# Kitware/SMQTK-Indexing

Measured on AMD Instinct MI355X. Metric: queries/sec, exact brute-force l2 kNN k=100 over 10000000x128 float32 (recall@100 = 1.0 by construction); scan HBM GB/s vs 8 TB/s peak, higher is better.
Workload: dtype f32 results (distances bit-identical to numpy float32); filter arithmetic int8 MFMA (i32 accumulation, measured per-row error bound), exact re-rank f32

## Files before the change

### smqtk_indexing_amd/csrc/sq_dense_exact.hpp

```cpp
#pragma once
#include "sq_pairwise.hpp"
#include "sq_select.hpp"

namespace sq {

typedef float f32x4 __attribute__((ext_vector_type(4)));
typedef float f32x16 __attribute__((ext_vector_type(16)));

__device__ __forceinline__ float np_sqdist_f32(const float* __restrict__ x, const float* __restrict__ q, int d, int j8) {
    auto term = [x, q](int i) {
        const float t = __fsub_rn(x[i], q[i]);
        return __fmul_rn(t, t);
    };
    return np_pairwise_sum<float>(term, d, j8);
}

__device__ __forceinline__ float sqrt_rn_f32(float v) {
    return (float)sqrt((double)v);
}

__device__ __forceinline__ double cosine_dist_f64(double dot, double nx2, double nq2) {
    double c = __ddiv_rn(dot, __dmul_rn(sqrt(nq2), sqrt(nx2)));
    if (fabs(c) > 1.0) c = copysign(1.0, c);
    double dm = 1.0 - c;
// ... 747 lines not shown
        __syncthreads();
        if (threadIdx.x == 0) {
            double tot = 0.0;
            for (int w = 0; w < (T >> 6); ++w) tot += red[w];
            qn2_out[q] = tot;
            cnt[q] = 0u;
            if (q == 0) *oflag = 0u;
            for (int p = nq + q; p < nq_pad; p += gridDim.x) {
                qn2_out[p] = 0.0;
                thr_out[p] = -__builtin_inff();
                cnt[p] = 0u;
            }
        }
        __syncthreads();
    }
    __device__ __forceinline__ float operator()(int q, float t) const {
        if (traw_out) traw_out[q] = t;
        if (!(t < __builtin_inff())) return t;
        double slack;
        if (cosine) {
            slack = 2.0 * fb.eps_cos + 1e-8;
        } else {
            const double Q = qn2[q];
            const double gamma = 1.0 - 2.0 * fb.alpha - fb.eps_b;
            const double c = fb.beta * Q + (double)t;
            const double disc = Q + gamma * c;
            double rho = (sqrt(Q) + sqrt(disc > 0.0 ? disc : 0.0)) / gamma;
            double rho2 = rho * rho * (1.0 + 1e-9);
            if (rho2 > fb.xn2_max) rho2 = fb.xn2_max;
            slack = (2.0 * fb.alpha + fb.eps_b) * rho2 + 2.0 * fb.beta * Q + 4e-6 * fabs((double)t + Q);
        }
        float r = (float)((double)t + slack);
        if ((double)r < (double)t + slack) r = __uint_as_float(__float_as_uint(r) + (r >= 0.f ? 1 : -1));
        return r;
    }
};

struct DenseCallPtrs {
    const float* q;
    void* out_dist;
    long long* out_idx;
};

struct DenseFinalizeL2 {
    const u32* cnt;
    u32 cap;
    int kk;
    long long id_base;
    const float* thr;
    const double* qn2;
    double beta;
    int certify;
    float* out_dist;
    long long* out_idx;
    u32* status;
    u32* cnt_out;
    const u32* overflow;
    int q0;
    ExactGroup sel = ExactGroup{{0, 0, 0, 0, 0, 0, 0, 0}, 0};
    const int* qmap = nullptr;
    const float2* lin = nullptr;
    const u32* thr2k = nullptr;
    int cnt_shift = 0;
    const DenseCallPtrs* ind = nullptr;
    __device__ __forceinline__ void operator()(int ql, const u64* sorted, int k) const {
        const int q = qmap ? qmap[ql] : (sel.count ? sel.idx[ql] : q0 + ql);
        const int qa = qmap ? ql : q;
        float* out_dist = ind ? static_cast<float*>(ind->out_dist) : this->out_dist;
        long long* out_idx = ind ? ind->out_idx : this->out_idx;
        for (int j = threadIdx.x; j < k; j += blockDim.x) {
            const u64 key = sorted[j];
            const bool pad = key == ~0ull;
            out_dist[(long long)q * k + j] = pad ? __builtin_inff() : unordered_f32((u32)(key >> 32));
            out_idx[(long long)q * k + j] = pad ? -1ll : id_base + (long long)(key & 0xffffffffull);
        }
        if (threadIdx.x == 0) {
            u32 st = 0;
            const u32 c = cnt[(long long)((sel.count || qmap) ? ql : q) << cnt_shift];
            if (certify) {
                if (c > cap || (overflow && *overflow)) st |= 1u;
                if (c < (u32)kk) st |= 4u;
                if (st == 0 && certify == 1) {
                    const double dk = (double)unordered_f32((u32)(sorted[kk - 1] >> 32));
                    const u32 t2k = thr2k ? thr2k[(long long)qa << cnt_shift] : 0u;
                    const double t = t2k ? (double)unordered_f32(t2k) : (double)thr[qa];
                    const double lo2 = t + qn2[qa] * (1.0 - beta) - (lin ? (double)lin[qa].y : 0.0);
                    const double bound = lo2 > 0.0 ? sqrt(lo2) * (1.0 - 1e-6) : 0.0;
                    if (!(t == (double)__builtin_inff()) && !(dk < bound)) st |= 2u;
                }
            }
            status[q] = st;
            if (cnt_out) cnt_out[q] = c;
        }
    }
};

struct DenseFinalizeCos {
    const u32* cnt;
    u32 cap;
    int kk;
    long long id_base;
    const float* thr;
    double eps;
    int certify;
    double* out_dist;
    long long* out_idx;
    u32* status;
    u32* cnt_out;
    const u32* overflow;
    int q0;
    ExactGroup sel = ExactGroup{{0, 0, 0, 0, 0, 0, 0, 0}, 0};
    const float2* lin = nullptr;
    const u32* thr2k = nullptr;
    int cnt_shift = 0;
    const DenseCallPtrs* ind = nullptr;
    const int* qmap = nullptr;
    __device__ __forceinline__ void operator()(int ql, const K128* sorted, int k) const {
        const int q = qmap ? qmap[ql] : (sel.count ? sel.idx[ql] : q0 + ql);
        const int qa = qmap ? ql : q;
        double* out_dist = ind ? static_cast<double*>(ind->out_dist) : this->out_dist;
        long long* out_idx = ind ? ind->out_idx : this->out_idx;
        for (int j = threadIdx.x; j < k; j += blockDim.x) {
            const K128 key = sorted[j];
            const bool pad = key.hi == ~0ull && key.lo == ~0ull;
            out_dist[(long long)q * k + j] = pad ? (double)__builtin_inff() : unordered_f64(key.hi);
            out_idx[(long long)q * k + j] = pad ? -1ll : id_base + (long long)(key.lo & 0xffffffffull);
        }
        if (threadIdx.x == 0) {
            u32 st = 0;
            const u32 c = cnt[(long long)((sel.count || qmap) ? ql : q) << cnt_shift];
            if (certify) {
                if (c > cap || (overflow && *overflow)) st |= 1u;
                if (c < (u32)kk) st |= 4u;
                if (st == 0 && certify == 1) {
                    const double dk = unordered_f64(sorted[kk - 1].hi);
                    const u32 t2k = thr2k ? thr2k[(long long)qa << cnt_shift] : 0u;
                    const double t = t2k ? (double)unordered_f32(t2k) : (double)thr[qa];
                    double smax = -t + (lin ? (double)lin[qa].y : eps);
                    smax = smax > 1.0 ? 1.0 : (smax < -1.0 ? -1.0 : smax);
                    const double bound = 2.0 * acos(smax) / 3.141592653589793 - 1e-9;
                    if (!(t == (double)__builtin_inff()) && !(dk < bound)) st |= 2u;
                }
            }
            status[q] = st;
            if (cnt_out) cnt_out[q] = c;
        }
    }
};

}
```

### smqtk_indexing_amd/csrc/sq_dense_i8.hpp

```cpp
#pragma once
#include "sq_dense_scan.hpp"

namespace sq {

typedef int i32x4 __attribute__((ext_vector_type(4)));
typedef int i32x16 __attribute__((ext_vector_type(16)));

template <int KS>
struct I8Geom {
    static constexpr int ROW_BYTES = KS * 32;
    static constexpr int UNIT_ROWS = KS == 4 ? 64 : 32;
    static constexpr int TILES = UNIT_ROWS / 32;
    static constexpr int UNIT_BYTES = UNIT_ROWS * ROW_BYTES;
    static constexpr int SLOT_BYTES = UNIT_BYTES + 256;
    static constexpr int WAVES = KS <= 8 ? 8 : 4;
    static constexpr int NSTAGE = 2;
    static constexpr int PIECES = UNIT_BYTES / 1024;
    static constexpr int SAMPLES_PER_UNIT = 2 * TILES;
};
static constexpr int I8_MAX_ROW_BYTES = 512;
__host__ __device__ constexpr int i8_row_bytes(int d) { return d <= 128 ? 128 : (d <= 256 ? 256 : 512); }
__host__ __device__ constexpr int i8_unit_rows(int row_bytes) { return row_bytes == 128 ? 64 : 32; }

__device__ __forceinline__ float i8_element(float v, const float* __restrict__ center, int k, bool cosine, double inv_norm) {
// ... 288 lines not shown
    par_out = make_float2((float)unit, real ? ef : 0.f);
    qn2_out = real ? Q : 0.0;
}

template <int EPL>
static __global__ __launch_bounds__(64) void dense8_prep_queries_kernel(const float* __restrict__ q, int nq, int d,
                                                                         const float* __restrict__ center, double dx, double r_max,
                                                                         double x_max, signed char* __restrict__ qs8,
                                                                         float2* __restrict__ par, double* __restrict__ qn2,
                                                                         float* __restrict__ thr, u32* __restrict__ cnt,
                                                                         u32* __restrict__ oflag, float* __restrict__ q_al, int ldq,
                                                                         const DenseCallPtrs* __restrict__ ind, int cosine, int plane_rows) {
    constexpr int row_bytes = EPL * 64;
    if (ind) q = ind->q;
    const int qi = blockIdx.x * 4 + (threadIdx.x >> 4), t = threadIdx.x & 15;
    if (t == 0) {
        thr[qi] = qi < nq ? -__builtin_inff() : __builtin_nanf("");
        cnt[qi] = 0u;
        if (qi == 0) *oflag = 0u;
    }
    if (qi < nq)
        for (int i = t; i < ldq; i += 16) q_al[(long long)qi * ldq + i] = i < d ? q[(long long)qi * d + i] : 0.f;
    float2 pr;
    double Q;
    dense8_prep_query_row<EPL>(q + (long long)qi * d, qi < nq, d, center, dx, r_max, x_max, cosine,
                               qs8 + (long long)qi * row_bytes, qs8 + (long long)(plane_rows + qi) * row_bytes, pr, Q);
    if (t == 0) {
        par[qi] = pr;
        qn2[qi] = Q;
    }
}

struct Dense8ThrPost {
    const float2* par;
    const double* qn2;
    __device__ __forceinline__ void prologue(int, double*) const {}
    __device__ __forceinline__ float operator()(int q, float t) const {
        if (!(t < __builtin_inff())) return t;
        if (!(par[q].y < __builtin_inff())) return __builtin_nanf("");
        const double tt = (double)t + 2.0 * (double)par[q].y + 4e-6 * fabs((double)t + qn2[q]);
        float r = (float)tt;
        if ((double)r < tt) r = __uint_as_float(__float_as_uint(r) + (r >= 0.f ? 1 : -1));
        return r;
    }
};

struct Dense8ScanArgs {
    const signed char* scan8;
    const float* nrow;
    long long n;
    long long n_units;
    const signed char* qs8;
    const float2* par;
    const float* thr;
    uint2* wave_out;
    u32* wave_cnt;
    u32 wave_cap;
    float* sample_out;
    long long ns;
    long long unit_step;
    long long n_sel;
    int nrb;
    int nt;
    long long nt_from_row;
    int nqt;
    int plane_rows;
    int debug;
    float* wave_score;
    u32* hist;
};

template <int KS>
__device__ __forceinline__ int i8_swz(int c, int r) {
    if constexpr (KS == 4) return c ^ ((r >> 1) & 7);
    return (c & ~15) | ((c & 15) ^ (r & 15));
}

enum { I8_EMIT = 0, I8_SAMPLE = 1, I8_LANEMIN = 2, I8_EMIT_H = 3 };

static constexpr int I8_HIST_BINS = 64;
static constexpr int I8_CNT_SHIFT = 5;
static constexpr int I8_HIST_WORDS = TILE_ROWS * I8_HIST_BINS + (TILE_ROWS << I8_CNT_SHIFT);

template <int WAVES>
__device__ __forceinline__ void dense8_hist_flush(u32* lds_hist, u32* __restrict__ ghist) {
    constexpr int PER = TILE_ROWS * I8_HIST_BINS / WAVES;
    const int lane = threadIdx.x & 63;
    const int wave = __builtin_amdgcn_readfirstlane(threadIdx.x >> 6);
#pragma unroll
    for (int i = 0; i < PER / 64; ++i) {
        const int b = wave * PER + i * 64 + lane;
        const u32 v = __hip_atomic_exchange(lds_hist + b, 0u, __ATOMIC_RELAXED, __HIP_MEMORY_SCOPE_WORKGROUP);
        if (v) __hip_atomic_fetch_add(ghist + b, v, __ATOMIC_RELAXED, __HIP_MEMORY_SCOPE_AGENT);
    }
}

template <int KS, int MODE>
__device__ __forceinline__ void dense8_stream(const Dense8ScanArgs& a, unsigned char* smem, const i32x4 (&bq)[KS], const i32x4 (&bl)[KS],
                                              float unit_lo, float thr_l, u32& wcount, float& smin, u32* lds_ticket,
                                              float inv_w_l = 0.f, u32* lds_hist = nullptr) {
    using G = I8Geom<KS>;
    constexpr bool SAMPLE = MODE == I8_SAMPLE || MODE == I8_LANEMIN;
    const int lane = threadIdx.x & 63;
    const int wave = __builtin_amdgcn_readfirstlane(threadIdx.x >> 6);
    const int r31 = lane & 31, h = lane >> 5;
    const u32 lds_base = (u32)(uintptr_t)smem;
    const u32 ring_base = lds_base + (u32)wave * (G::NSTAGE * G::SLOT_BYTES);
    const unsigned char* ring_ptr = smem + wave * (G::NSTAGE * G::SLOT_BYTES);
    const long long wave_id = (long long)blockIdx.x * G::WAVES + wave;
    const long long nwaves = (long long)a.nrb * G::WAVES;
    uint2* wout = a.wave_out + wave_id * a.wave_cap;
    float* wsc = MODE == I8_EMIT_H ? a.wave_score + wave_id * a.wave_cap : nullptr;
    u32* hist_l = MODE == I8_EMIT_H ? lds_hist + r31 * I8_HIST_BINS : nullptr;

    const long long wg_first = (long long)blockIdx.x * G::WAVES;
    auto take_unit = [&]() __attribute__((always_inline)) -> long long {
        u32 t = 0;
        if (lane == 0) t = __hip_atomic_fetch_add(lds_ticket, 1u, __ATOMIC_RELAXED, __HIP_MEMORY_SCOPE_WORKGROUP);
        t = (u32)__builtin_amdgcn_readfirstlane((int)t);
        const long long u = wg_first + (long long)(t % G::WAVES) + (long long)(t / G::WAVES) * nwaves;
        return u < a.n_sel ? u : -1ll;
    };
    const long long my_units = wave_id < a.n_sel ? (a.n_sel - wave_id + nwaves - 1) / nwaves : 0;
    u32 voff[G::PIECES];
#pragma unroll
    for (int j = 0; j < G::PIECES; ++j) {
        const int lin = j * 1024 + lane * 16;
        const int r = lin / G::ROW_BYTES, cpos = (lin % G::ROW_BYTES) >> 4;
        voff[j] = (u32)(r * G::ROW_BYTES + i8_swz<KS>(cpos, r) * 16);
    }
    const u32 voff_n = (u32)lane * 4u;
    static_assert(G::NSTAGE == 2, "two ring slots: the units in flight are sel_even / sel_odd");
    long long issued = 0, sel_even = -1, sel_odd = -1;
    bool more = true;
    auto issue_next = [&]() __attribute__((always_inline)) {
        if (!more) return;
        const long long sel = take_unit();
        if (sel < 0) {
            more = false;
            return;
        }
        if (issued & 1) sel_odd = sel; else sel_even = sel;
        const long long unit_idx = sel * a.unit_step;
        const long long row0 = unit_idx * G::UNIT_ROWS;
        const u32 dst = ring_base + (u32)(issued % G::NSTAGE) * G::SLOT_BYTES;
        const unsigned char* base = reinterpret_cast<const unsigned char*>(a.scan8) + row0 * G::ROW_BYTES;
#pragma unroll
        for (int j = 0; j < G::PIECES; ++j) {
            if (a.nt && row0 >= a.nt_from_row)
                glds16<true>(base, voff[j], dst + (u32)j * 1024);
            else
                glds16<false>(base, voff[j], dst + (u32)j * 1024);
        }
        glds4(a.nrow + row0, voff_n, dst + G::UNIT_BYTES);
        ++issued;
    };
    for (int p = 0; p < G::NSTAGE; ++p) issue_next();
    const int flush_every = (int)(my_units >> 3) > 0 ? (int)(my_units >> 3) : 1;
    int to_flush = flush_every;

    for (long long it = 0; it < issued; ++it) {
        const long long sel = (it & 1) ? sel_odd : sel_even;
        const long long unit_idx = sel * a.unit_step;
        const long long row0 = unit_idx * G::UNIT_ROWS;
        wait_units_in_flight<G::NSTAGE, G::PIECES + 1>((int)(issued - it - 1));
        const unsigned char* sl = ring_ptr + (it % G::NSTAGE) * G::SLOT_BYTES;
        constexpr int KH = KS == 16 ? 8 : KS;
        i32x4 av[G::TILES][KH];
        f32x4 nr[G::TILES][4];
#pragma unroll
        for (int t = 0; t < G::TILES; ++t) {
            const int r = 32 * t + r31;
#pragma unroll
            for (int s = 0; s < KH; ++s)
                av[t][s] = *reinterpret_cast<const i32x4*>(sl + r * G::ROW_BYTES + i8_swz<KS>(2 * s + h, r) * 16);
#pragma unroll
            for (int c = 0; c < 4; ++c) nr[t][c] = *reinterpret_cast<const f32x4*>(sl + G::UNIT_BYTES + (32 * t + 8 * c + 4 * h) * 4);
        }
        asm volatile("s_waitcnt lgkmcnt(0)" ::: "memory");
        if constexpr (KS != 16) issue_next();
#pragma unroll
        for (int t = 0; t < G::TILES; ++t) {
            i32x16 acc, acl;
#pragma unroll
            for (int i = 0; i < 16; ++i) acc[i] = acl[i] = 0;
#pragma unroll
            for (int s = 0; s < KH; ++s) {
                acc = __builtin_amdgcn_mfma_i32_32x32x32_i8(av[t][s], bq[s], acc, 0, 0, 0);
                acl = __builtin_amdgcn_mfma_i32_32x32x32_i8(av[t][s], bl[s], acl, 0, 0, 0);
            }
            if constexpr (KS == 16) {
#pragma unroll
                for (int s = 0; s < KH; ++s)
                    av[t][s] = *reinterpret_cast<const i32x4*>(sl + r31 * G::ROW_BYTES + i8_swz<KS>(2 * (KH + s) + h, r31) * 16);
                asm volatile("s_waitcnt lgkmcnt(0)" ::: "memory");
                issue_next();
#pragma unroll
                for (int s = 0; s < KH; ++s) {
                    acc = __builtin_amdgcn_mfma_i32_32x32x32_i8(av[t][s], bq[KH + s], acc, 0, 0, 0);
                    acl = __builtin_amdgcn_mfma_i32_32x32x32_i8(av[t][s], bl[KH + s], acl, 0, 0, 0);
                }
            }
            if (a.debug & 1024) {
                if (acc[0] == 0x7fffffff && acl[5] == 0x7ffffffe) wcount += 1;
                continue;
            }
            float sc[16];
#pragma unroll
            for (int i = 0; i < 16; ++i) {
                float nv = nr[t][i >> 2][i & 3];
                if constexpr (SAMPLE) nv = nv == -__builtin_inff() ? __builtin_inff() : nv;
                sc[i] = __fmaf_rn((float)((acc[i] << 8) + acl[i]), unit_lo, nv);
            }
            float m = sc[0];
#pragma unroll
            for (int i = 1; i < 16; ++i) m = fminf(m, sc[i]);
            if constexpr (MODE == I8_LANEMIN) {
                smin = fminf(smin, m);
            } else if constexpr (MODE == I8_SAMPLE) {
                a.sample_out[(long long)r31 * a.ns + sel * G::SAMPLES_PER_UNIT + t * 2 + h] = m;
            } else {
                const u64 hit = __ballot(m <= thr_l);
                if (hit != 0) {
                    u32 mask = 0;
#pragma unroll
                    for (int i = 0; i < 16; ++i) mask |= (sc[i] <= thr_l ? 1u : 0u) << i;
                    const u64 bal = __ballot(mask != 0);
                    if (mask) {
                        const u32 pos = wcount + __builtin_amdgcn_mbcnt_hi((u32)(bal >> 32), __builtin_amdgcn_mbcnt_lo((u32)bal, 0u));
                        if (pos < a.wave_cap) {
                            wout[pos] = make_uint2((u32)(row0 + 32 * t + 4 * h), (mask << 16) | (u32)r31);
                            if constexpr (MODE == I8_EMIT_H) wsc[pos] = m;
                        }
                        if constexpr (MODE == I8_EMIT_H) {
                            if (m > -__builtin_inff()) {
                                const int bin = min((int)((thr_l - m) * inv_w_l), I8_HIST_BINS - 1);
                                __hip_atomic_fetch_add(hist_l + bin, 1u, __ATOMIC_RELAXED, __HIP_MEMORY_SCOPE_WORKGROUP);
                            }
                        }
                    }
                    wcount += (u32)__popcll(bal);
                }
            }
        }
        if constexpr (MODE == I8_EMIT_H) {
            if (--to_flush == 0) {
                to_flush = flush_every;
                dense8_hist_flush<G::WAVES>(lds_hist, a.hist);
            }
        }
    }
}

template <int KS>
__device__ __forceinline__ void dense8_load_planes(const signed char* planes, i32x4 (&bq)[KS], i32x4 (&bl)[KS]) {
    using G = I8Geom<KS>;
    const int lane = threadIdx.x & 63, r31 = lane & 31, h = lane >> 5;
#pragma unroll
    for (int s = 0; s < KS; ++s) {
        bq[s] = *reinterpret_cast<const i32x4*>(planes + r31 * G::ROW_BYTES + (2 * s + h) * 16);
        bl[s] = *reinterpret_cast<const i32x4*>(planes + (TILE_ROWS + r31) * G::ROW_BYTES + (2 * s + h) * 16);
    }
#pragma unroll
    for (int s = 0; s < KS; ++s) asm volatile("" : "+v"(bq[s]), "+v"(bl[s]));
}

template <int KS, bool SAMPLE>
__global__ __launch_bounds__(I8Geom<KS>::WAVES * 64, KS == 16 ? 1 : 2) void dense8_scan_kernel(Dense8ScanArgs a) {
    using G = I8Geom<KS>;
    extern __shared__ __attribute__((aligned(16))) unsigned char smem[];
    const int lane = threadIdx.x & 63;
    const int wave = __builtin_amdgcn_readfirstlane(threadIdx.x >> 6);
    const int r31 = lane & 31;
    i32x4 bq[KS], bl[KS];
    dense8_load_planes<KS>(a.qs8, bq, bl);
    float unit_lo = a.par[r31].x * 0.00390625f;
    float thr_l = SAMPLE ? 0.f : a.thr[r31];
    asm volatile("" : "+v"(unit_lo), "+v"(thr_l));
    u32 wcount = 0;
    float smin = 0.f;
    __shared__ u32 s_unit_ticket;
    if (threadIdx.x == 0) s_unit_ticket = 0u;
    __syncthreads();
    dense8_stream<KS, SAMPLE ? I8_SAMPLE : I8_EMIT>(a, smem, bq, bl, unit_lo, thr_l, wcount, smin, &s_unit_ticket);
    if constexpr (!SAMPLE) {
        if (lane == 0) {
            const long long wave_id = (long long)blockIdx.x * G::WAVES + wave;
            a.wave_cnt[2 * wave_id] = wcount;
            a.wave_cnt[2 * wave_id + 1] = 0u;
        }
    }
}


struct Dense8HeadArgs {
    Dense8ScanArgs s;
    const float* q;
    int nq, d;
    const float* center;
    double dx, r_max, x_max;
    int cosine;
    double* qn2;
    u32* cnt;
    u32* oflag;
    float* q_al;
    int ldq;
    const DenseCallPtrs* ind;
    float* lane_min;
    int keep;
    int kk;
};

template <int VM, int NQ>
__device__ __forceinline__ void wave_kth_smallest(const float* __restrict__ vals, long long stride, int M, int k, float (&out)[NQ]) {
    const int lane = threadIdx.x & 63;
    constexpr u32 KINF = 0xff800000u;
    u32 key[NQ][VM];
    u32 prefix[NQ];
    u32 xall = 0u;
#pragma unroll
    for (int n = 0; n < NQ; ++n) {
        u32 kmin = KINF, kmax = 0u;
#pragma unroll
        for (int j = 0; j < VM; ++j) {
            const int i = j * 64 + lane;
            u32 kv = ordered_f32(vals[n * stride + (i < M ? i : 0)]);
            kv = (i < M && kv < KINF) ? kv : KINF;
            key[n][j] = kv;
            kmin = kv < kmin ? kv : kmin;
            kmax = kv > kmax ? kv : kmax;
        }
        for (int o = 32; o > 0; o >>= 1) {
            const u32 a = (u32)__shfl_xor((int)kmin, o), b = (u32)__shfl_xor((int)kmax, o);
            kmin = a < kmin ? a : kmin;
            kmax = b > kmax ? b : kmax;
        }
        prefix[n] = __builtin_amdgcn_readfirstlane(kmin);
        xall |= __builtin_amdgcn_readfirstlane(kmin ^ kmax);
    }
    if (xall != 0u) {
        const int top = 31 - __clz((int)xall);
#pragma unroll
        for (int n = 0; n < NQ; ++n) prefix[n] &= ~((2u << top) - 1u);
        for (int b = top; b >= 0; --b) {
#pragma unroll
            for (int n = 0; n < NQ; ++n) {
                const u32 cand = prefix[n] | ((1u << b) - 1u);
                u32 c = 0;
#pragma unroll
                for (int j = 0; j < VM; ++j) c += (u32)__popcll(__ballot(key[n][j] <= cand));
                if (c < (u32)k) prefix[n] |= 1u << b;
            }
        }
    }
#pragma unroll
    for (int n = 0; n < NQ; ++n) {
        float r = unordered_f32(prefix[n]);
        if (prefix[n] >= KINF) {
            u32 c = 0;
#pragma unroll
            for (int j = 0; j < VM; ++j) c += (u32)__popcll(__ballot(key[n][j] < KINF));
            if (c < (u32)k) r = __builtin_inff();
        }
        out[n] = r;
    }
}

template <int KS>
__global__ __launch_bounds__(I8Geom<KS>::WAVES * 64, KS == 16 ? 1 : 2) void dense8_head_kernel(Dense8HeadArgs ha) {
    using G = I8Geom<KS>;
    constexpr int VB = G::WAVES * 2;
    extern __shared__ __attribute__((aligned(16))) unsigned char smem[];
    __shared__ float2 s_par[TILE_ROWS];
    __shared__ double s_qn2[TILE_ROWS];
    __shared__ float s_lm[TILE_ROWS][16];
    __shared__ u32 s_ticket, s_unit_ticket;
    if (threadIdx.x == 0) s_unit_ticket = 0u;
    const Dense8ScanArgs& a = ha.s;
    const int lane = threadIdx.x & 63;
    const int wave = __builtin_amdgcn_readfirstlane(threadIdx.x >> 6);
    const int r31 = lane & 31, h = lane >> 5;
    const float* q = ha.ind ? ha.ind->q : ha.q;
    const bool first = blockIdx.x == 0;
    signed char* planes = reinterpret_cast<signed char*>(smem);
#pragma unroll
    for (int rnd = 0; rnd < TILE_ROWS / (4 * G::WAVES); ++rnd) {
        const int qi = rnd * 4 * G::WAVES + wave * 4 + (lane >> 4);
        float2 pr;
        double Q;
        dense8_prep_query_row<KS / 2>(q + (long long)qi * ha.d, qi < ha.nq, ha.d, ha.center, ha.dx, ha.r_max, ha.x_max, ha.cosine,
                                      planes + qi * G::ROW_BYTES, planes + (TILE_ROWS + qi) * G::ROW_BYTES, pr, Q);
        if ((lane & 15) == 0) {
            s_par[qi] = pr;
            s_qn2[qi] = Q;
        }
        if (first) {
            if ((lane & 15) == 0) {
                const_cast<float2*>(a.par)[qi] = pr;
                ha.qn2[qi] = Q;
                ha.cnt[qi << I8_CNT_SHIFT] = 0u;
                if (qi == 0) ha.oflag[0] = 0u;
            }
            if (qi < ha.nq)
                for (int i = lane & 15; i < ha.ldq; i += 16) ha.q_al[(long long)qi * ha.ldq + i] = i < ha.d ? q[(long long)qi * ha.d + i] : 0.f;
        }
    }
    __syncthreads();
    i32x4 bq[KS], bl[KS];
    dense8_load_planes<KS>(planes, bq, bl);
    float unit_lo = s_par[r31].x * 0.00390625f;
    asm volatile("" : "+v"(unit_lo));
    if (first) {
        signed char* gp = const_cast<signed char*>(a.qs8);
        for (int i = threadIdx.x; i < 2 * TILE_ROWS * G::ROW_BYTES / 16; i += G::WAVES * 64)
            reinterpret_cast<uint4*>(gp)[i] = reinterpret_cast<const uint4*>(planes)[i];
        for (int i = threadIdx.x; i < I8_HIST_WORDS; i += G::WAVES * 64) a.hist[i] = 0u;
    }
    asm volatile("s_waitcnt vmcnt(0) lgkmcnt(0)" ::: "memory");
    __syncthreads();
    u32 wcount = 0;
    float smin = __builtin_inff();
    if (!(a.debug & 4096)) dense8_stream<KS, I8_LANEMIN>(a, smem, bq, bl, unit_lo, 0.f, wcount, smin, &s_unit_ticket);
    s_lm[r31][(wave * 2 + h) & 15] = smin;
    if (VB < 16 && wave == 0 && h == 0)
        for (int i = VB; i < 16; ++i) s_lm[r31][i] = __builtin_inff();
    __syncthreads();
    const int nb = (int)gridDim.x, keep = ha.keep, M = nb * keep;
#pragma unroll
    for (int rnd = 0; rnd < TILE_ROWS / (4 * G::WAVES); ++rnd) {
        const int qi = rnd * 4 * G::WAVES + wave * 4 + (lane >> 4), l16 = lane & 15;
        float v = s_lm[qi][l16];
#pragma unroll
        for (int kk2 = 2; kk2 <= 16; kk2 <<= 1)
#pragma unroll
            for (int j = kk2 >> 1; j > 0; j >>= 1) {
                const float o = __shfl_xor(v, j);
                const bool up = (l16 & kk2) == 0, lower = (l16 & j) == 0;
                v = (lower == up) ? fminf(v, o) : fmaxf(v, o);
            }
        if (l16 < keep) ha.lane_min[(long long)qi * M + (long long)blockIdx.x * keep + l16] = v;
    }
    asm volatile("s_waitcnt vmcnt(0)" ::: "memory");
    __syncthreads();
    if (threadIdx.x == 0) {
        __threadfence();
        const u32 t = atomicAdd(&ha.oflag[1], 1u);
        if (t == gridDim.x - 1) {
            __threadfence();
            ha.oflag[1] = 0u;
        }
        s_ticket = t;
    }
    __syncthreads();
    if (s_ticket != gridDim.x - 1) return;
    float* thr = const_cast<float*>(a.thr);
    const Dense8ThrPost post{s_par, s_qn2};
#pragma unroll
    for (int rnd = 0; rnd < TILE_ROWS / (4 * G::WAVES); ++rnd) {
        const int q0 = rnd * 4 * G::WAVES + wave * 4;
        float ts[4] = {-__builtin_inff(), -__builtin_inff(), -__builtin_inff(), -__builtin_inff()};
        if (q0 < ha.nq && !(a.debug & 2048)) {
            const float* v = ha.lane_min + (long long)q0 * M;
            if (M <= 256)
                wave_kth_smallest<4, 4>(v, M, M, ha.kk, ts);
            else if (M <= 512)
                wave_kth_smallest<8, 4>(v, M, M, ha.kk, ts);
            else if (M <= 1024)
                wave_kth_smallest<16, 4>(v, M, M, ha.kk, ts);
            else {
#pragma unroll
                for (int j = 0; j < 4; ++j) {
                    float one[1];
                    wave_kth_smallest<32, 1>(v + (long long)j * M, M, M, ha.kk, one);
                    ts[j] = one[0];
                }
            }
        }
#pragma unroll
        for (int j = 0; j < 4; ++j) {
            const float t = q0 + j < ha.nq ? post(q0 + j, ts[j]) : __builtin_nanf("");
            if (lane == 0) thr[q0 + j] = t;
        }
    }
}

struct Dense8TailArgs {
    const float* db;
    long long ld;
    int d;
    const float* q_al;
    int ldq, nq;
    void* keys;
    u32* cnt;
    u32 cap;
    u32* overflow;
    const double* nx64;
    const double* nq64;
    int debug;
    const double* qn2;
    int kk;
    int tighten;
    long long* clk;
};
static constexpr int I8_TAIL_QROWS_BYTES = 32 * (156 + 4) * 4;
static constexpr int I8_TAIL_LIST = 2048;
static constexpr int I8_TAIL_RERANK_BYTES = I8_TAIL_QROWS_BYTES + 3 * RERANK_MAX_GROUP * 4 + 8 * 32 * RERANK_STAGE_STRIDE * 4;
static constexpr int I8_TAIL_LDS_BYTES = I8_TAIL_RERANK_BYTES + I8_TAIL_LIST * 8 + TILE_ROWS * 4 + 16;

template <int KS, bool COSINE>
__global__ __launch_bounds__(I8Geom<KS>::WAVES * 64, KS == 16 ? 1 : 2) void dense8_body_kernel(Dense8ScanArgs a, Dense8TailArgs ta) {
    using G = I8Geom<KS>;
    static_assert(I8_TAIL_LDS_BYTES <= G::WAVES * G::NSTAGE * G::SLOT_BYTES, "the re-rank works in the ring's LDS");
    extern __shared__ __attribute__((aligned(16))) unsigned char smem[];
    __shared__ u32 s_hist8[TILE_ROWS * I8_HIST_BINS];
    __shared__ u32 s_wcnt[G::WAVES];
    __shared__ u32 s_unit_ticket;
    __shared__ float s_thr1[TILE_ROWS], s_eq[TILE_ROWS];
    __shared__ double s_qn2b[TILE_ROWS];
    __shared__ float2 s_parb[TILE_ROWS];
    if (threadIdx.x == 0) s_unit_ticket = 0u;
    if (threadIdx.x < TILE_ROWS) {
        s_thr1[threadIdx.x] = a.thr[threadIdx.x];
        s_parb[threadIdx.x] = a.par[threadIdx.x];
        s_eq[threadIdx.x] = a.par[threadIdx.x].y;
        s_qn2b[threadIdx.x] = ta.qn2[threadIdx.x];
    }
    const int lane = threadIdx.x & 63;
    const int wave = __builtin_amdgcn_readfirstlane(threadIdx.x >> 6);
    const int r31 = lane & 31;
    for (int i = threadIdx.x; i < TILE_ROWS * I8_HIST_BINS; i += G::WAVES * 64) s_hist8[i] = 0u;
    long long* clk = ta.clk ? ta.clk + (long long)blockIdx.x * 8 : nullptr;
    if (clk && threadIdx.x == 0) {
        clk[0] = (long long)wall_clock64();
        clk[1] = 0x7fffffffffffffffll;
    }
    __syncthreads();
    i32x4 bq[KS], bl[KS];
    dense8_load_planes<KS>(a.qs8, bq, bl);
    float unit_lo = a.par[r31].x * 0.00390625f;
    float thr_l = a.thr[r31];
    const float eq_l = a.par[r31].y;
    float inv_w_l = (eq_l > 0.f && eq_l < __builtin_inff()) ? 2.f / eq_l : 0.f;
    if (!(inv_w_l < 3.0e38f)) inv_w_l = 0.f;
    asm volatile("" : "+v"(unit_lo), "+v"(thr_l), "+v"(inv_w_l));
    u32 wcount = 0;
    float smin = 0.f;
    dense8_stream<KS, I8_EMIT_H>(a, smem, bq, bl, unit_lo, thr_l, wcount, smin, &s_unit_ticket, inv_w_l, s_hist8);
    const long long w0 = (long long)blockIdx.x * G::WAVES;
    if (lane == 0) {
        a.wave_cnt[2 * (w0 + wave)] = wcount;
        a.wave_cnt[2 * (w0 + wave) + 1] = 0u;
        s_wcnt[wave] = wcount;
        if (clk) atomicMin((unsigned long long*)(clk + 1), (unsigned long long)wall_clock64());
    }
    asm volatile("s_waitcnt vmcnt(0) lgkmcnt(0)" ::: "memory");
    __builtin_amdgcn_fence(__ATOMIC_RELEASE, "workgroup");
    __syncthreads();
    __builtin_amdgcn_fence(__ATOMIC_ACQUIRE, "workgroup");
    if (clk && threadIdx.x == 0) clk[2] = (long long)wall_clock64();
    float* fl = reinterpret_cast<float*>(smem);
    u32* su = reinterpret_cast<u32*>(smem + I8_TAIL_QROWS_BYTES);
    RerankLds L{fl, su, su + RERANK_MAX_GROUP, su + 2 * RERANK_MAX_GROUP,
                COSINE ? reinterpret_cast<float*>(smem + I8_TAIL_QROWS_BYTES + 3 * RERANK_MAX_GROUP * 4) : nullptr};
    {
        uint2* s_list = reinterpret_cast<uint2*>(smem + I8_TAIL_RERANK_BYTES);
        float* s_thr2 = reinterpret_cast<float*>(smem + I8_TAIL_RERANK_BYTES + I8_TAIL_LIST * 8);
        u32* s_npass = reinterpret_cast<u32*>(s_thr2 + TILE_ROWS);
        static_assert(I8_HIST_BINS == 64, "one lane per bin");
        bool any = false;
#pragma unroll
        for (int wi = 0; wi < G::WAVES; ++wi) any = any || s_wcnt[wi] != 0u;
        const Dense8ThrPost post{s_parb, s_qn2b};
        constexpr int NQW = TILE_ROWS / G::WAVES;
        u32 hc[NQW];
        if (ta.tighten && any) {
#pragma unroll
            for (int j = 0; j < NQW; ++j) {
                const int qi = (j >> 2) * 4 * G::WAVES + wave * 4 + (j & 3);
                hc[j] = __hip_atomic_load(a.hist + qi * I8_HIST_BINS + lane, __ATOMIC_RELAXED, __HIP_MEMORY_SCOPE_AGENT);
            }
#pragma unroll
            for (int j = 0; j < NQW; ++j) {
                const int qi = (j >> 2) * 4 * G::WAVES + wave * 4 + (j & 3);
                hc[j] += s_hist8[qi * I8_HIST_BINS + lane];
            }
        }
#pragma unroll
        for (int rnd = 0; rnd < TILE_ROWS / (4 * G::WAVES); ++rnd) {
#pragma unroll
            for (int j = 0; j < 4; ++j) {
                const int qi = rnd * 4 * G::WAVES + wave * 4 + j;
                const float t1 = s_thr1[qi];
                float t2 = t1;
                if (ta.tighten && any && qi < ta.nq && t1 < __builtin_inff() && t1 > -__builtin_inff()) {
                    u32 c = hc[rnd * 4 + j];
#pragma unroll
                    for (int o = 1; o < 64; o <<= 1) {
                        const u32 up = (u32)__shfl_down((int)c, o);
                        c += lane + o < 64 ? up : 0u;
                    }
                    const u64 reach = __ballot(c >= (u32)ta.kk);
                    const float eq = s_eq[qi];
                    if (reach != 0ull && eq > 0.f && eq < __builtin_inff()) {
                        const int jb = 63 - __clzll((long long)reach);
                        const float inv_w = 2.f / eq;
                        if (inv_w < 3.0e38f) {
                            const double t8 = (double)t1 - (double)jb / (double)inv_w * (1.0 - 1e-6);
                            float t8f = (float)t8;
                            if ((double)t8f < t8) t8f = __uint_as_float(__float_as_uint(t8f) + (t8f >= 0.f ? 1 : -1));
                            const float cand = post(qi, t8f);
                            if (cand < t2) t2 = cand;
                        }
                    }
                    if (lane == 0) atomicMax(a.hist + TILE_ROWS * I8_HIST_BINS + (qi << I8_CNT_SHIFT), ordered_f32(t2));
                }
                if (lane == 0) s_thr2[qi] = t2;
            }
        }
        if (ta.tighten) {
            L.scores = a.wave_score;
            L.thr2 = s_thr2;
            L.list = s_list;
            L.npass = s_npass;
            L.list_cap = I8_TAIL_LIST;
        }
        L.seg_cnt = s_wcnt;
        L.cnt_shift = I8_CNT_SHIFT;
        __syncthreads();
        if (clk && threadIdx.x == 0) clk[3] = (long long)wall_clock64();
        if (ta.tighten) dense8_hist_flush<G::WAVES>(s_hist8, a.hist);
    }
    using K = typename std::conditional<COSINE, K128, u64>::type;
    rerank_block<K, COSINE>(ta.db, ta.ld, ta.d, ta.q_al, ta.ldq, ta.nq, TILE_ROWS, a.wave_out, a.wave_cnt, a.wave_cap,
                            (long long)a.nrb * G::WAVES, G::WAVES, static_cast<K*>(ta.keys), ta.cnt, ta.cap, ta.overflow, ta.nx64,
                            ta.nq64, ta.debug, w0, L);
    if (clk) {
        asm volatile("s_waitcnt vmcnt(0) lgkmcnt(0)" ::: "memory");
        __syncthreads();
        if (threadIdx.x == 0) clk[4] = (long long)wall_clock64();
    }
}

template <int QT, bool SAMPLE>
__global__ __launch_bounds__(512, 2) void dense8_scan_mt_kernel(Dense8ScanArgs a) {
    using G = I8Geom<4>;
    extern __shared__ __attribute__((aligned(16))) unsigned char smem[];
    const int lane = threadIdx.x & 63;
    const int wave = __builtin_amdgcn_readfirstlane(threadIdx.x >> 6);
    const int r31 = lane & 31, h = lane >> 5;
    const u32 lds_base = (u32)(uintptr_t)smem;
    const u32 ring_base = lds_base + (u32)wave * (G::NSTAGE * G::SLOT_BYTES);
    const unsigned char* ring_ptr = smem + wave * (G::NSTAGE * G::SLOT_BYTES);
    const long long wave_id = (long long)blockIdx.x * G::WAVES + wave;
    uint2* wout = a.wave_out + wave_id * a.wave_cap;
    const int L = blockIdx.x;
    int grp, rb;
    if (a.nqt > 1) {
        const int xcd = L & 7, j = L >> 3;
        grp = j % a.nqt;
        rb = (j / a.nqt) * 8 + xcd;
    } else {
        grp = 0;
        rb = L;
    }
    const int q_first = grp * QT * TILE_ROWS;
    const long long rwave = (long long)rb * G::WAVES + wave, nwaves = (long long)a.nrb * G::WAVES;

    i32x4 bq[QT][4], bl[QT][4];
    float unit_lo[QT], thr_l[QT];
#pragma unroll
    for (int g = 0; g < QT; ++g) {
        const int qg = q_first + g * TILE_ROWS + r31;
#pragma unroll
        for (int s = 0; s < 4; ++s) {
            bq[g][s] = *reinterpret_cast<const i32x4*>(a.qs8 + (long long)qg * G::ROW_BYTES + (2 * s + h) * 16);
            bl[g][s] = *reinterpret_cast<const i32x4*>(a.qs8 + (long long)(a.plane_rows + qg) * G::ROW_BYTES + (2 * s + h) * 16);
        }
        unit_lo[g] = a.par[qg].x * 0.00390625f;
        thr_l[g] = SAMPLE ? 0.f : a.thr[qg];
        asm volatile("" : "+v"(unit_lo[g]), "+v"(thr_l[g]));
#pragma unroll
        for (int s = 0; s < 4; ++s) asm volatile("" : "+v"(bq[g][s]), "+v"(bl[g][s]));
    }

    const long long my_units = rwave < a.n_sel ? (a.n_sel - rwave + nwaves - 1) / nwaves : 0;
    u32 voff[G::PIECES];
#pragma unroll
    for (int j = 0; j < G::PIECES; ++j) {
        const int r = 8 * j + (lane >> 3);
        voff[j] = (u32)(r * G::ROW_BYTES + i8_swz<4>(lane & 7, r) * 16);
    }
    const u32 voff_n = (u32)lane * 4u;
    long long issued = 0;
    auto issue_next = [&]() __attribute__((always_inline)) {
        if (issued >= my_units) return;
        const long long unit_idx = (rwave + issued * nwaves) * a.unit_step;
        const long long row0 = unit_idx * G::UNIT_ROWS;
// ... 81 lines not shown
```

Before: 149,100.

## Stage emit writes and histogram flush across DMA refill, prefetch tickets, pad LDS hist

The int8 scan loop now fetches the next unit ticket one step ahead, computes addresses in 32-bit, and issues unit DMA through an m0-based helper with pre-biased offsets. Candidate emits and the global histogram atomics are held in registers and written out at the next refill point, so those stores overlap the in-flight loads instead of sitting on the MFMA path. The LDS histogram rows gain one padding word to avoid bank conflicts. The per-query tightened threshold changes from atomicMax with zero init to atomicMin with all-ones init, and the finalize sentinel is updated to match. This is a semantic change to how per-block thresholds combine.

Measured after the change: 151,100 (median of 6 runs). +1.3%, better.

```diff
diff --git a/smqtk_indexing_amd/csrc/sq_dense_exact.hpp b/smqtk_indexing_amd/csrc/sq_dense_exact.hpp
--- a/smqtk_indexing_amd/csrc/sq_dense_exact.hpp
+++ b/smqtk_indexing_amd/csrc/sq_dense_exact.hpp
@@ -853,8 +853,8 @@
                 if (c < (u32)kk) st |= 4u;
                 if (st == 0 && certify == 1) {
                     const double dk = (double)unordered_f32((u32)(sorted[kk - 1] >> 32));
-                    const u32 t2k = thr2k ? thr2k[(long long)qa << cnt_shift] : 0u;
-                    const double t = t2k ? (double)unordered_f32(t2k) : (double)thr[qa];
+                    const u32 t2k = thr2k ? thr2k[(long long)qa << cnt_shift] : 0xffffffffu;
+                    const double t = t2k != 0xffffffffu ? (double)unordered_f32(t2k) : (double)thr[qa];
                     const double lo2 = t + qn2[qa] * (1.0 - beta) - (lin ? (double)lin[qa].y : 0.0);
                     const double bound = lo2 > 0.0 ? sqrt(lo2) * (1.0 - 1e-6) : 0.0;
                     if (!(t == (double)__builtin_inff()) && !(dk < bound)) st |= 2u;
@@ -905,8 +905,8 @@
                 if (c < (u32)kk) st |= 4u;
                 if (st == 0 && certify == 1) {
                     const double dk = unordered_f64(sorted[kk - 1].hi);
-                    const u32 t2k = thr2k ? thr2k[(long long)qa << cnt_shift] : 0u;
-                    const double t = t2k ? (double)unordered_f32(t2k) : (double)thr[qa];
+                    const u32 t2k = thr2k ? thr2k[(long long)qa << cnt_shift] : 0xffffffffu;
+                    const double t = t2k != 0xffffffffu ? (double)unordered_f32(t2k) : (double)thr[qa];
                     double smax = -t + (lin ? (double)lin[qa].y : eps);
                     smax = smax > 1.0 ? 1.0 : (smax < -1.0 ? -1.0 : smax);
                     const double bound = 2.0 * acos(smax) / 3.141592653589793 - 1e-9;
diff --git a/smqtk_indexing_amd/csrc/sq_dense_i8.hpp b/smqtk_indexing_amd/csrc/sq_dense_i8.hpp
--- a/smqtk_indexing_amd/csrc/sq_dense_i8.hpp
+++ b/smqtk_indexing_amd/csrc/sq_dense_i8.hpp
@@ -394,17 +394,48 @@
 static constexpr int I8_CNT_SHIFT = 5;
 static constexpr int I8_HIST_WORDS = TILE_ROWS * I8_HIST_BINS + (TILE_ROWS << I8_CNT_SHIFT);
 
+static constexpr int I8_HIST_STRIDE = I8_HIST_BINS + 1;
+
+template <int WAVES>
+struct Dense8HistShare {
+    static constexpr int PER = TILE_ROWS * I8_HIST_BINS / WAVES;
+    u32 v[PER / 64];
+    __device__ __forceinline__ void take(u32* lds_hist) {
+        const int lane = threadIdx.x & 63;
+        const int wave = __builtin_amdgcn_readfirstlane(threadIdx.x >> 6);
+#pragma unroll
+        for (int i = 0; i < PER / 64; ++i)
+            v[i] = __hip_atomic_exchange(lds_hist + (wave * (PER / 64) + i) * I8_HIST_STRIDE + lane, 0u, __ATOMIC_RELAXED,
+                                         __HIP_MEMORY_SCOPE_WORKGROUP);
+    }
+    __device__ __forceinline__ void add(u32* __restrict__ ghist) const {
+        const int lane = threadIdx.x & 63;
+        const int wave = __builtin_amdgcn_readfirstlane(threadIdx.x >> 6);
+#pragma unroll
+        for (int i = 0; i < PER / 64; ++i)
+            if (v[i]) __hip_atomic_fetch_add(ghist + wave * PER + i * 64 + lane, v[i], __ATOMIC_RELAXED, __HIP_MEMORY_SCOPE_AGENT);
+    }
+};
 template <int WAVES>
 __device__ __forceinline__ void dense8_hist_flush(u32* lds_hist, u32* __restrict__ ghist) {
-    constexpr int PER = TILE_ROWS * I8_HIST_BINS / WAVES;
-    const int lane = threadIdx.x & 63;
-    const int wave = __builtin_amdgcn_readfirstlane(threadIdx.x >> 6);
-#pragma unroll
-    for (int i = 0; i < PER / 64; ++i) {
-        const int b = wave * PER + i * 64 + lane;
-        const u32 v = __hip_atomic_exchange(lds_hist + b, 0u, __ATOMIC_RELAXED, __HIP_MEMORY_SCOPE_WORKGROUP);
-        if (v) __hip_atomic_fetch_add(ghist + b, v, __ATOMIC_RELAXED, __HIP_MEMORY_SCOPE_AGENT);
-    }
+    Dense8HistShare<WAVES> sh;
+    sh.take(lds_hist);
+    sh.add(ghist);
+}
+
+template <int PIECES, int UNIT_BYTES, bool NT>
+__device__ __forceinline__ void dense8_dma_unit(const unsigned char* base, const float* nrow0, const u32 (&voff)[PIECES], u32 voff_n,
+                                                u32 dst) {
+#pragma unroll
+    for (int j = 0; j < PIECES; ++j) {
+        static_for_one<8>(j & 7, [&](auto jj) __attribute__((always_inline)) {
+            constexpr int J = decltype(jj)::value;
+            if constexpr (J == 0) glds_set_m0(dst + (u32)(j >> 3) * 8192u + 4096u);
+            glds16_m0<J * 1024 - 4096, NT>(base, voff[j]);
+        });
+    }
+    glds_set_m0(dst + UNIT_BYTES);
+    glds4_m0<0>(nrow0, voff_n);
 }
 
 template <int KS, int MODE>
@@ -413,70 +444,104 @@
                                               float inv_w_l = 0.f, u32* lds_hist = nullptr) {
     using G = I8Geom<KS>;
     constexpr bool SAMPLE = MODE == I8_SAMPLE || MODE == I8_LANEMIN;
+    constexpr bool HIST = MODE == I8_EMIT_H;
     const int lane = threadIdx.x & 63;
     const int wave = __builtin_amdgcn_readfirstlane(threadIdx.x >> 6);
     const int r31 = lane & 31, h = lane >> 5;
     const u32 lds_base = (u32)(uintptr_t)smem;
     const u32 ring_base = lds_base + (u32)wave * (G::NSTAGE * G::SLOT_BYTES);
     const unsigned char* ring_ptr = smem + wave * (G::NSTAGE * G::SLOT_BYTES);
-    const long long wave_id = (long long)blockIdx.x * G::WAVES + wave;
-    const long long nwaves = (long long)a.nrb * G::WAVES;
-    uint2* wout = a.wave_out + wave_id * a.wave_cap;
-    float* wsc = MODE == I8_EMIT_H ? a.wave_score + wave_id * a.wave_cap : nullptr;
-    u32* hist_l = MODE == I8_EMIT_H ? lds_hist + r31 * I8_HIST_BINS : nullptr;
-
-    const long long wg_first = (long long)blockIdx.x * G::WAVES;
-    auto take_unit = [&]() __attribute__((always_inline)) -> long long {
-        u32 t = 0;
-        if (lane == 0) t = __hip_atomic_fetch_add(lds_ticket, 1u, __ATOMIC_RELAXED, __HIP_MEMORY_SCOPE_WORKGROUP);
-        t = (u32)__builtin_amdgcn_readfirstlane((int)t);
-        const long long u = wg_first + (long long)(t % G::WAVES) + (long long)(t / G::WAVES) * nwaves;
-        return u < a.n_sel ? u : -1ll;
+    const u32 wave_id = blockIdx.x * G::WAVES + (u32)wave;
+    const u32 nwaves = (u32)a.nrb * G::WAVES;
+    const u32 n_sel = (u32)a.n_sel, unit_step = (u32)a.unit_step;
+    const u32 nt_from = !a.nt ? 0xffffffffu : (a.nt_from_row >= 0xffffffffll ? 0xffffffffu : (u32)(a.nt_from_row > 0 ? a.nt_from_row : 0));
+    uint2* wout = a.wave_out + (long long)wave_id * a.wave_cap;
+    float* wsc = HIST ? a.wave_score + (long long)wave_id * a.wave_cap : nullptr;
+    u32* hist_l = HIST ? lds_hist + r31 * I8_HIST_STRIDE : nullptr;
+
+    const u32 wg_first = blockIdx.x * G::WAVES;
+    u32 t_pend = 0;
+    auto fetch_ticket = [&]() __attribute__((always_inline)) {
+        if (lane == 0) t_pend = __hip_atomic_fetch_add(lds_ticket, 1u, __ATOMIC_RELAXED, __HIP_MEMORY_SCOPE_WORKGROUP);
     };
-    const long long my_units = wave_id < a.n_sel ? (a.n_sel - wave_id + nwaves - 1) / nwaves : 0;
+    const u32 my_units = wave_id < n_sel ? (n_sel - wave_id + nwaves - 1) / nwaves : 0;
     u32 voff[G::PIECES];
 #pragma unroll
     for (int j = 0; j < G::PIECES; ++j) {
         const int lin = j * 1024 + lane * 16;
         const int r = lin / G::ROW_BYTES, cpos = (lin % G::ROW_BYTES) >> 4;
-        voff[j] = (u32)(r * G::ROW_BYTES + i8_swz<KS>(cpos, r) * 16);
+        voff[j] = (u32)(r * G::ROW_BYTES + i8_swz<KS>(cpos, r) * 16 - ((j & 7) * 1024 - 4096));
     }
     const u32 voff_n = (u32)lane * 4u;
     static_assert(G::NSTAGE == 2, "two ring slots: the units in flight are sel_even / sel_odd");
-    long long issued = 0, sel_even = -1, sel_odd = -1;
+    u32 issued = 0, sel_even = 0, sel_odd = 0;
     bool more = true;
+    fetch_ticket();
     auto issue_next = [&]() __attribute__((always_inline)) {
         if (!more) return;
-        const long long sel = take_unit();
-        if (sel < 0) {
+        const u32 t = (u32)__builtin_amdgcn_readfirstlane((int)t_pend);
+        const u32 sel = wg_first + t % G::WAVES + (t / G::WAVES) * nwaves;
+        if (sel >= n_sel) {
             more = false;
             return;
         }
+        fetch_ticket();
         if (issued & 1) sel_odd = sel; else sel_even = sel;
-        const long long unit_idx = sel * a.unit_step;
-        const long long row0 = unit_idx * G::UNIT_ROWS;
-        const u32 dst = ring_base + (u32)(issued % G::NSTAGE) * G::SLOT_BYTES;
-        const unsigned char* base = reinterpret_cast<const unsigned char*>(a.scan8) + row0 * G::ROW_BYTES;
-#pragma unroll
-        for (int j = 0; j < G::PIECES; ++j) {
-            if (a.nt && row0 >= a.nt_from_row)
-                glds16<true>(base, voff[j], dst + (u32)j * 1024);
-            else
-                glds16<false>(base, voff[j], dst + (u32)j * 1024);
-        }
-        glds4(a.nrow + row0, voff_n, dst + G::UNIT_BYTES);
+        const u32 row0 = sel * unit_step * G::UNIT_ROWS;
+        const u32 dst = ring_base + (issued & 1) * G::SLOT_BYTES;
+        const unsigned char* base = reinterpret_cast<const unsigned char*>(a.scan8) + (u64)row0 * G::ROW_BYTES;
+        if (row0 >= nt_from)
+            dense8_dma_unit<G::PIECES, G::UNIT_BYTES, true>(base, a.nrow + row0, voff, voff_n, dst);
+        else
+            dense8_dma_unit<G::PIECES, G::UNIT_BYTES, false>(base, a.nrow + row0, voff, voff_n, dst);
         ++issued;
     };
     for (int p = 0; p < G::NSTAGE; ++p) issue_next();
-    const int flush_every = (int)(my_units >> 3) > 0 ? (int)(my_units >> 3) : 1;
-    int to_flush = flush_every;
-
-    for (long long it = 0; it < issued; ++it) {
-        const long long sel = (it & 1) ? sel_odd : sel_even;
-        const long long unit_idx = sel * a.unit_step;
-        const long long row0 = unit_idx * G::UNIT_ROWS;
+    const u32 flush_every = (my_units >> 3) > 0 ? (my_units >> 3) : 1;
+    u32 to_flush = flush_every;
+
+    constexpr bool EMIT = !SAMPLE;
+    u32 st_pos[G::TILES], st_x[G::TILES], st_y[G::TILES];
+    float st_m[G::TILES];
+#pragma unroll
+    for (int t = 0; t < G::TILES; ++t) {
+        st_pos[t] = 0xffffffffu;
+        st_x[t] = st_y[t] = 0u;
+        st_m[t] = 0.f;
+    }
+    bool staged = false, flush_staged = false;
+    Dense8HistShare<G::WAVES> share;
+    auto write_staged = [&]() __attribute__((always_inline)) {
+        if constexpr (EMIT) {
+            if (staged) {
+#pragma unroll
+                for (int t = 0; t < G::TILES; ++t) {
+                    if (st_pos[t] != 0xffffffffu) {
+                        wout[st_pos[t]] = make_uint2(st_x[t], st_y[t]);
+                        if constexpr (HIST) wsc[st_pos[t]] = st_m[t];
+                    }
+                    st_pos[t] = 0xffffffffu;
+                }
+                staged = false;
+            }
+            if constexpr (HIST) {
+                if (flush_staged) {
+                    share.add(a.hist);
+                    flush_staged = false;
+                }
+            }
+        }
+    };
+    auto refill = [&]() __attribute__((always_inline)) {
+        write_staged();
+        issue_next();
+    };
+
+    for (u32 it = 0; it < issued; ++it) {
+        const u32 sel = (it & 1) ? sel_odd : sel_even;
+        const u32 row0 = sel * unit_step * G::UNIT_ROWS;
         wait_units_in_flight<G::NSTAGE, G::PIECES + 1>((int)(issued - it - 1));
-        const unsigned char* sl = ring_ptr + (it % G::NSTAGE) * G::SLOT_BYTES;
+        const unsigned char* sl = ring_ptr + (it & 1) * G::SLOT_BYTES;
         constexpr int KH = KS == 16 ? 8 : KS;
         i32x4 av[G::TILES][KH];
         f32x4 nr[G::TILES][4];
@@ -490,7 +555,7 @@
             for (int c = 0; c < 4; ++c) nr[t][c] = *reinterpret_cast<const f32x4*>(sl + G::UNIT_BYTES + (32 * t + 8 * c + 4 * h) * 4);
         }
         asm volatile("s_waitcnt lgkmcnt(0)" ::: "memory");
-        if constexpr (KS != 16) issue_next();
+        if constexpr (KS != 16) refill();
 #pragma unroll
         for (int t = 0; t < G::TILES; ++t) {
             i32x16 acc, acl;
@@ -506,7 +571,7 @@
                 for (int s = 0; s < KH; ++s)
                     av[t][s] = *reinterpret_cast<const i32x4*>(sl + r31 * G::ROW_BYTES + i8_swz<KS>(2 * (KH + s) + h, r31) * 16);
                 asm volatile("s_waitcnt lgkmcnt(0)" ::: "memory");
-                issue_next();
+                refill();
 #pragma unroll
                 for (int s = 0; s < KH; ++s) {
                     acc = __builtin_amdgcn_mfma_i32_32x32x32_i8(av[t][s], bq[KH + s], acc, 0, 0, 0);
@@ -530,7 +595,7 @@
             if constexpr (MODE == I8_LANEMIN) {
                 smin = fminf(smin, m);
             } else if constexpr (MODE == I8_SAMPLE) {
-                a.sample_out[(long long)r31 * a.ns + sel * G::SAMPLES_PER_UNIT + t * 2 + h] = m;
+                a.sample_out[(long long)r31 * a.ns + (long long)sel * G::SAMPLES_PER_UNIT + t * 2 + h] = m;
             } else {
                 const u64 hit = __ballot(m <= thr_l);
                 if (hit != 0) {
@@ -541,27 +606,32 @@
                     if (mask) {
                         const u32 pos = wcount + __builtin_amdgcn_mbcnt_hi((u32)(bal >> 32), __builtin_amdgcn_mbcnt_lo((u32)bal, 0u));
                         if (pos < a.wave_cap) {
-                            wout[pos] = make_uint2((u32)(row0 + 32 * t + 4 * h), (mask << 16) | (u32)r31);
-                            if constexpr (MODE == I8_EMIT_H) wsc[pos] = m;
+                            st_pos[t] = pos;
+                            st_x[t] = row0 + 32 * t + 4 * h;
+                            st_y[t] = (mask << 16) | (u32)r31;
+                            st_m[t] = m;
                         }
-                        if constexpr (MODE == I8_EMIT_H) {
+                        if constexpr (HIST) {
                             if (m > -__builtin_inff()) {
                                 const int bin = min((int)((thr_l - m) * inv_w_l), I8_HIST_BINS - 1);
                                 __hip_atomic_fetch_add(hist_l + bin, 1u, __ATOMIC_RELAXED, __HIP_MEMORY_SCOPE_WORKGROUP);
                             }
                         }
                     }
+                    staged = true;
                     wcount += (u32)__popcll(bal);
                 }
             }
         }
-        if constexpr (MODE == I8_EMIT_H) {
+        if constexpr (HIST) {
             if (--to_flush == 0) {
                 to_flush = flush_every;
-                dense8_hist_flush<G::WAVES>(lds_hist, a.hist);
-            }
-        }
-    }
+                share.take(lds_hist);
+                flush_staged = true;
+            }
+        }
+    }
+    write_staged();
 }
 
 template <int KS>
@@ -726,7 +796,8 @@
         signed char* gp = const_cast<signed char*>(a.qs8);
         for (int i = threadIdx.x; i < 2 * TILE_ROWS * G::ROW_BYTES / 16; i += G::WAVES * 64)
             reinterpret_cast<uint4*>(gp)[i] = reinterpret_cast<const uint4*>(planes)[i];
-        for (int i = threadIdx.x; i < I8_HIST_WORDS; i += G::WAVES * 64) a.hist[i] = 0u;
+        for (int i = threadIdx.x; i < I8_HIST_WORDS; i += G::WAVES * 64)
+            a.hist[i] = i < TILE_ROWS * I8_HIST_BINS ? 0u : 0xffffffffu;
     }
     asm volatile("s_waitcnt vmcnt(0) lgkmcnt(0)" ::: "memory");
     __syncthreads();
@@ -824,7 +895,7 @@
     using G = I8Geom<KS>;
     static_assert(I8_TAIL_LDS_BYTES <= G::WAVES * G::NSTAGE * G::SLOT_BYTES, "the re-rank works in the ring's LDS");
     extern __shared__ __attribute__((aligned(16))) unsigned char smem[];
-    __shared__ u32 s_hist8[TILE_ROWS * I8_HIST_BINS];
+    __shared__ u32 s_hist8[TILE_ROWS * I8_HIST_STRIDE];
     __shared__ u32 s_wcnt[G::WAVES];
     __shared__ u32 s_unit_ticket;
     __shared__ float s_thr1[TILE_ROWS], s_eq[TILE_ROWS];
@@ -840,7 +911,7 @@
     const int lane = threadIdx.x & 63;
     const int wave = __builtin_amdgcn_readfirstlane(threadIdx.x >> 6);
     const int r31 = lane & 31;
-    for (int i = threadIdx.x; i < TILE_ROWS * I8_HIST_BINS; i += G::WAVES * 64) s_hist8[i] = 0u;
+    for (int i = threadIdx.x; i < TILE_ROWS * I8_HIST_STRIDE; i += G::WAVES * 64) s_hist8[i] = 0u;
     long long* clk = ta.clk ? ta.clk + (long long)blockIdx.x * 8 : nullptr;
     if (clk && threadIdx.x == 0) {
         clk[0] = (long long)wall_clock64();
@@ -894,7 +965,7 @@
 #pragma unroll
             for (int j = 0; j < NQW; ++j) {
                 const int qi = (j >> 2) * 4 * G::WAVES + wave * 4 + (j & 3);
-                hc[j] += s_hist8[qi * I8_HIST_BINS + lane];
+                hc[j] += s_hist8[qi * I8_HIST_STRIDE + lane];
             }
         }
 #pragma unroll
@@ -924,7 +995,7 @@
                             if (cand < t2) t2 = cand;
                         }
                     }
-                    if (lane == 0) atomicMax(a.hist + TILE_ROWS * I8_HIST_BINS + (qi << I8_CNT_SHIFT), ordered_f32(t2));
+                    if (lane == 0) atomicMin(a.hist + TILE_ROWS * I8_HIST_BINS + (qi << I8_CNT_SHIFT), ordered_f32(t2));
                 }
                 if (lane == 0) s_thr2[qi] = t2;
             }
```
